# GestaltCogTeam/STEP

Measured on AMD Instinct MI355X. Metric: training windows/sec on PEMS04, horizon-12 MAE parity, 1/2/4/8 MI355X, higher is better.
Workload: dtype f16 (TSFormer Q/K/weights) + bf16 (P, V, GraphWaveNet / graph-learner GEMMs) operands, f32 accumulate

## Files before the change

include/step_hip.h:

```cpp
#ifndef STEP_HIP_H
#define STEP_HIP_H

#include <stdint.h>

#ifdef __cplusplus
extern "C" {
#endif

const char* step_last_error(void);
int step_abi_version(void);

typedef struct StepGemm {
    int M, N, K, batch;
    const void* A; long sam, sak, sab; int a_bf16;
    const void* B; long sbk, sbn, sbb; int b_bf16;
    float* C; long ldc, scn, scb;
    float alpha;
    int accumulate;
    const float* bias; int relu;
    int splitk;
    int a_kblk; long a_kstride;
    int b_kblk; long b_kstride;
    int b_nblk; long b_nstride;
    int c_nblk; long c_nstride;
// ... 8 lines not shown
int step_gemm(const StepGemm* g, void* stream);

#define STEP_ENC_F16 1
#define STEP_ENC_ALWAYS_RESHIFT 2
#define STEP_ENC_RANGE_FLAG 4
#define STEP_ENC_WORKGROUPS(n) (((n) & 0xffff) << 8)
int step_tsformer_encode(const float* series, int S, int L, const void* wpack, long wpack_bytes,
                         int depth, int flags, uint16_t* hidden_bf16, float* hidden_f32, float* last_f32,
                         float* sqnorm_part, float dropout_p, const uint64_t* drop_pool, long pool_words, uint64_t seed,
                         unsigned int* fallback_count, void* stream);
int step_dropout_pool_fill(uint64_t* pool, long words, float dropout_p, uint64_t seed, void* stream);
long step_tsformer_dropout_words(int L, int depth);

int step_pack_long_history(const float* x, int B, int L, int N, int C, int ch, float* out, void* stream);
int step_gather_windows(const float* data, int T, int N, int C, int ch, const long* t0, int B, int L, int H,
                        float* long_series, float* hist, float* fut, void* stream);

long step_knn_workspace_bytes(int B, int N, int F);
int step_knn_graph(const uint16_t* hidden, const float* sqnorm_part, int B, int N, int F, int k_total,
                   float* sim, float* adj, void* work, long work_bytes, void* stream);
int step_topk_mask(const float* sim, int B, int N, int k_total, float* adj, void* work, long work_bytes,
                   void* stream);

typedef struct StepDglParams {
    float *conv1_w, *conv1_b;
    float *conv2_w, *conv2_b;
    float *fc_w, *fc_b;
    float *bn1_w, *bn1_b, *bn1_rm, *bn1_rv;
    float *bn2_w, *bn2_b, *bn2_rm, *bn2_rv;
    float *bn3_w, *bn3_b, *bn3_rm, *bn3_rv;
    float *fc_out_w, *fc_out_b;
    float *fc_cat_w, *fc_cat_b;
    int gemm_bf16;
} StepDglParams;

long step_dgl_global_saved_floats(int N, int T);
long step_dgl_global_work_floats(int N, int T, int backward);
int step_dgl_global_forward(const float* series_nt, int N, int T, const StepDglParams* p, int training,
                            float momentum, float* saved, float* work, float* g, void* stream);
int step_dgl_global_backward(const float* series_nt, int N, int T, const StepDglParams* p, const float* saved,
                             const float* dg, float* work, const StepDglParams* grads, void* stream);
#define STEP_DGL_FRESH_FC_GRAD 16
int step_dgl_global_backward_phase(const float* series_nt, int N, int T, const StepDglParams* p, const float* saved,
                             const float* dg, float* work, const StepDglParams* grads, int phase, void* stream);

typedef struct StepDglShard { int own1; double count1, count2; } StepDglShard;
int step_dgl_global_forward_shard(const float* series_slice, int N, int Ts, const StepDglParams* p, int training, float momentum,
                                  float* saved, float* work, double* sums, float* g, const StepDglShard* shard, int phase,
                                  void* stream);
int step_dgl_global_backward_shard(const float* series_slice, int N, int Ts, const StepDglParams* p, const float* saved,
                                   const float* dg, float* work, const StepDglParams* grads, const StepDglShard* shard, int phase,
                                   void* stream);
long step_dgl_global_offset(int N, int T, int item);

long step_dgl_edges_saved_floats(int B, int N);
long step_dgl_edges_work_floats(int N);
long step_dgl_edges_theta_offset(int N);
int step_dgl_edges_forward(const float* g, int N, int B, const StepDglParams* p, const float* u, uint64_t seed,
                           float temperature, float* saved, float* theta_out, float* adj_out, void* stream);
int step_dgl_edges_backward(const float* g, int N, int B, const StepDglParams* p, const float* saved,
                            const float* dtheta, const float* dadj, float temperature, float* work,
                            const StepDglParams* grads, float* dg, void* aux_stream, void* stream);

typedef struct StepGwnetParams {
    float *nodevec1, *nodevec2;
    float *start_w, *start_b;
    float *filter_w[8], *filter_b[8];
    float *gate_w[8], *gate_b[8];
    float *skip_w[8], *skip_b[8];
    float *bn_w[8], *bn_b[8], *bn_rm[8], *bn_rv[8];
    float *gconv_w[8], *gconv_b[8];
    float *fc_his0_w, *fc_his0_b, *fc_his2_w, *fc_his2_b;
    float *end1_w, *end1_b, *end2_w, *end2_b;
    int gemm_bf16;
} StepGwnetParams;

long step_gwnet_saved_floats(int B, int N, int dropout);
long step_gwnet_work_floats(int B, int N, int backward);
long step_gwnet_saved_offset(int B, int N, int dropout, int item, int layer);
int step_gwnet_forward(const float* hist, int B, int N, int Cin, const float* hidden_last, const float* adj,
                       const StepGwnetParams* p, int training, float dropout_p, uint64_t seed, float momentum,
                       float* saved, float* work, float* pred, void* stream);
int step_gwnet_forward_phase(const float* hist, int B, int N, int Cin, const float* hidden_last, const float* adj,
                             const StepGwnetParams* p, int training, float dropout_p, uint64_t seed, float momentum,
                             float* saved, float* work, float* pred, int phase, void* stream);
int step_gwnet_backward(const float* hist, int B, int N, int Cin, const float* hidden_last, const StepGwnetParams* p,
                        const float* saved, float* work, const float* dpred, const StepGwnetParams* grads,
                        float* dadj, int dropout, void* aux_stream, void* leaf_stream, void* stream);

int step_pt_dropout(const float* x, float* y, long n, float p, uint64_t seed, uint32_t site, void* stream);
int step_pt_ffn_hidden_fwd(const float* x, const float* w1, const float* b1, long R, float p, uint64_t seed, uint32_t site,
                           uint16_t* hidden, void* stream);
int step_pt_ffn_hidden_bwd(const float* dy, const float* w2, const uint16_t* hidden, long R, float p, uint16_t* dhidden, void* stream);
int step_pt_colsum_bf16(const uint16_t* x, long rows, int cols, float* out, void* stream);
long step_pt_rows_linear_pack_bytes(int nkc, int nog);
int step_pt_rows_linear_pack(const float* w, long swo, long swi, int nkc, int nog, const float* bias, void* pack, void* stream);
int step_pt_rows_linear(const void* x, int x_bf16, long R, const void* pack, int nkc, int nog, void* y, int y_bf16, int accumulate, void* stream);
int step_pt_layer_pack(const float* wi, const float* bi, const float* wo, const float* bo, const float* w1, const float* b1, const float* w2,
                       const float* b2, void* ffn, void* qkv, void* o, void* da, void* dx, void* stream);
long step_pt_proj_wgrad_ws_floats(long R);
int step_pt_proj_wgrad(const float* x, const uint16_t* dqkv, const float* dov, const uint16_t* a, long R, float* ws, float* dwi, float* dbi, float* dwo,
                       void* stream);
int step_pt_ffn_fused_fwd_ln(const float* h1, long R, const void* pack, float p, const uint64_t* pool, long pool_words, uint64_t seed, uint32_t site_hidden,
                             uint32_t site_out, const float* gamma, const float* beta, float* pre, float* y, float* stats, void* stream);
int step_pt_rows_linear_ln(const uint16_t* x, long R, const void* pack, const float* res, float p, uint64_t seed, uint32_t site, const float* gamma,
                           const float* beta, float* pre, float* y, float* stats, void* stream);
// ... 129 lines not shown
```

step_amd/_lib.py:

```python
import ctypes
import os

import torch

_HERE = os.path.dirname(os.path.abspath(__file__))
LIB_PATH = os.environ.get("STEP_HIP_LIB") or os.path.join(_HERE, "libstep_hip.so")

_vp, _i, _l, _f, _u64 = ctypes.c_void_p, ctypes.c_int, ctypes.c_long, ctypes.c_float, ctypes.c_uint64


class StepGemm(ctypes.Structure):
    _fields_ = [("M", _i), ("N", _i), ("K", _i), ("batch", _i),
                ("A", _vp), ("sam", _l), ("sak", _l), ("sab", _l), ("a_bf16", _i),
                ("B", _vp), ("sbk", _l), ("sbn", _l), ("sbb", _l), ("b_bf16", _i),
                ("C", _vp), ("ldc", _l), ("scn", _l), ("scb", _l),
                ("alpha", _f), ("accumulate", _i), ("bias", _vp), ("relu", _i), ("splitk", _i),
                ("a_kblk", _i), ("a_kstride", _l), ("b_kblk", _i), ("b_kstride", _l),
                ("b_nblk", _i), ("b_nstride", _l), ("c_nblk", _i), ("c_nstride", _l),
                ("a_kscale", _vp), ("a_kshift", _vp), ("a_kperiod", _i),
                ("batch0", _i), ("sab1", _l), ("sbb1", _l), ("scb1", _l), ("compute_bf16", _i), ("a_rowsum", _vp), ("c_nscale", _vp), ("c_nshift", _vp), ("c_mvec", _vp),
                ("c_nperiod", _i), ("splitk_ws", _vp), ("splitk_ws_floats", _l)]


class StepDglParams(ctypes.Structure):
    NAMES = ["conv1_w", "conv1_b", "conv2_w", "conv2_b", "fc_w", "fc_b",
             "bn1_w", "bn1_b", "bn1_rm", "bn1_rv", "bn2_w", "bn2_b", "bn2_rm", "bn2_rv",
             "bn3_w", "bn3_b", "bn3_rm", "bn3_rv", "fc_out_w", "fc_out_b", "fc_cat_w", "fc_cat_b"]
    _fields_ = [(n, _vp) for n in NAMES] + [("gemm_bf16", _i)]


class StepGwnetParams(ctypes.Structure):
    _fields_ = [("nodevec1", _vp), ("nodevec2", _vp), ("start_w", _vp), ("start_b", _vp),
                ("filter_w", _vp * 8), ("filter_b", _vp * 8), ("gate_w", _vp * 8), ("gate_b", _vp * 8),
                ("skip_w", _vp * 8), ("skip_b", _vp * 8),
                ("bn_w", _vp * 8), ("bn_b", _vp * 8), ("bn_rm", _vp * 8), ("bn_rv", _vp * 8),
                ("gconv_w", _vp * 8), ("gconv_b", _vp * 8),
                ("fc_his0_w", _vp), ("fc_his0_b", _vp), ("fc_his2_w", _vp), ("fc_his2_b", _vp),
                ("end1_w", _vp), ("end1_b", _vp), ("end2_w", _vp), ("end2_b", _vp), ("gemm_bf16", _i)]


_PD = ctypes.POINTER(StepDglParams)


class StepDynState(ctypes.Structure):
    _fields_ = [("seed_xor", ctypes.c_uint64), ("adam_step", ctypes.c_int32), ("lr", _f), ("gsl_coef", _f), ("reserved", _f)]


class StepDglShard(ctypes.Structure):
    _fields_ = [("own1", ctypes.c_int), ("count1", ctypes.c_double), ("count2", ctypes.c_double)]


_PS = ctypes.POINTER(StepDglShard)
_PG = ctypes.POINTER(StepGwnetParams)

_SIGS = {
    "step_last_error": (ctypes.c_char_p, []),
    "step_abi_version": (_i, []),
    "step_gemm": (_i, [ctypes.POINTER(StepGemm), _vp]),
    "step_tsformer_encode": (_i, [_vp, _i, _i, _vp, _l, _i, _i, _vp, _vp, _vp, _vp, _f, _vp, _l, _u64, _vp, _vp]),
    "step_dropout_pool_fill": (_i, [_vp, _l, _f, _u64, _vp]),
    "step_tsformer_dropout_words": (_l, [_i, _i]),
    "step_gather_windows": (_i, [_vp, _i, _i, _i, _i, _vp, _i, _i, _i, _vp, _vp, _vp, _vp]),
    "step_pack_long_history": (_i, [_vp, _i, _i, _i, _i, _i, _vp, _vp]),
    "step_knn_workspace_bytes": (_l, [_i, _i, _i]),
    "step_knn_graph": (_i, [_vp, _vp, _i, _i, _i, _i, _vp, _vp, _vp, _l, _vp]),
    "step_topk_mask": (_i, [_vp, _i, _i, _i, _vp, _vp, _l, _vp]),
    "step_selftest_mfma": (_i, [_vp, _vp]),
    "step_streams_concurrent": (_i, [_vp, _vp, ctypes.POINTER(_i)]),
    "step_dgl_global_saved_floats": (_l, [_i, _i]),
    "step_dgl_global_work_floats": (_l, [_i, _i, _i]),
    "step_dgl_global_forward": (_i, [_vp, _i, _i, _PD, _i, _f, _vp, _vp, _vp, _vp]),
    "step_dgl_global_backward": (_i, [_vp, _i, _i, _PD, _vp, _vp, _vp, _PD, _vp]),
    "step_dgl_global_backward_phase": (_i, [_vp, _i, _i, _PD, _vp, _vp, _vp, _PD, _i, _vp]),
    "step_dgl_global_forward_shard": (_i, [_vp, _i, _i, _PD, _i, _f, _vp, _vp, _vp, _vp, _PS, _i, _vp]),
    "step_dgl_global_backward_shard": (_i, [_vp, _i, _i, _PD, _vp, _vp, _vp, _PD, _PS, _i, _vp]),
    "step_dgl_global_offset": (_l, [_i, _i, _i]),
    "step_dgl_edges_saved_floats": (_l, [_i, _i]),
    "step_dgl_edges_work_floats": (_l, [_i]),
    "step_dgl_edges_theta_offset": (_l, [_i]),
    "step_dgl_edges_forward": (_i, [_vp, _i, _i, _PD, _vp, _u64, _f, _vp, _vp, _vp, _vp]),
    "step_dgl_edges_backward": (_i, [_vp, _i, _i, _PD, _vp, _vp, _vp, _f, _vp, _PD, _vp, _vp, _vp]),
    "step_gwnet_saved_floats": (_l, [_i, _i, _i]),
    "step_gwnet_work_floats": (_l, [_i, _i, _i]),
    "step_gwnet_saved_offset": (_l, [_i, _i, _i, _i, _i]),
    "step_gwnet_forward": (_i, [_vp, _i, _i, _i, _vp, _vp, _PG, _i, _f, _u64, _f, _vp, _vp, _vp, _vp]),
    "step_gwnet_forward_phase": (_i, [_vp, _i, _i, _i, _vp, _vp, _PG, _i, _f, _u64, _f, _vp, _vp, _vp, _i, _vp]),
    "step_gwnet_backward": (_i, [_vp, _i, _i, _i, _vp, _PG, _vp, _vp, _vp, _PG, _vp, _i, _vp, _vp, _vp]),
    "step_pt_dropout": (_i, [_vp, _vp, _l, _f, _u64, ctypes.c_uint32, _vp]),
    "step_pt_ffn_hidden_fwd": (_i, [_vp, _vp, _vp, _l, _f, _u64, ctypes.c_uint32, _vp, _vp]),
    "step_pt_ffn_hidden_bwd": (_i, [_vp, _vp, _vp, _l, _f, _vp, _vp]),
    "step_pt_colsum_bf16": (_i, [_vp, _l, _i, _vp, _vp]),
    "step_pt_rows_linear_pack_bytes": (_l, [_i, _i]),
    "step_pt_rows_linear_pack": (_i, [_vp, _l, _l, _i, _i, _vp, _vp, _vp]),
    "step_pt_rows_linear": (_i, [_vp, _i, _l, _vp, _i, _i, _vp, _i, _i, _vp]),
    "step_pt_layer_pack": (_i, [_vp] * 14),
    "step_pt_proj_wgrad_ws_floats": (_l, [_l]),
    "step_pt_proj_wgrad": (_i, [_vp, _vp, _vp, _vp, _l, _vp, _vp, _vp, _vp, _vp]),
    "step_pt_ffn_fused_fwd_ln": (_i, [_vp, _l, _vp, _f, _vp, _l, _u64, ctypes.c_uint32, ctypes.c_uint32, _vp, _vp, _vp, _vp, _vp, _vp]),
    "step_pt_rows_linear_ln": (_i, [_vp, _l, _vp, _vp, _f, _u64, ctypes.c_uint32, _vp, _vp, _vp, _vp, _vp, _vp]),
    "step_pt_embed_unmasked_fwd": (_i, [_vp, _vp, _vp, _vp, _vp, _l, _i, _i, _f, _u64, ctypes.c_uint32, _vp, _vp]),
    "step_pt_embed_unmasked_bwd": (_i, [_vp, _vp, _vp, _l, _i, _i, _f, _u64, ctypes.c_uint32, _vp, _vp, _vp, _vp]),
    "step_pt_dec_input_bwd_sums": (_i, [_vp, _l, _i, _i, _f, _u64, ctypes.c_uint32, _vp, _vp, _vp, _vp, _vp]),
    "step_pt_ffn_pack_bytes": (_l, []),
    "step_pt_ffn_wgrad_workgroups": (_l, [_l]),
    "step_pt_ffn_wgrad_ws_floats": (_l, [_l]),
    "step_pt_ffn_pack": (_i, [_vp, _vp, _vp, _vp, _vp, _vp]),
    "step_pt_ffn_fused_fwd": (_i, [_vp, _l, _vp, _f, _vp, _l, _u64, ctypes.c_uint32, _vp, _vp]),
    "step_pt_ffn_fused_bwd_data": (_i, [_vp, _vp, _l, _vp, _f, _vp, _l, _u64, ctypes.c_uint32, _vp, _vp]),
    "step_pt_ffn_fused_bwd_weights": (_i, [_vp, _vp, _l, _vp, _vp, _f, _vp, _l, _u64, ctypes.c_uint32, _vp, _vp, _vp, _vp, _vp]),
    "step_pt_add_layernorm_fwd": (_i, [_vp, _vp, _l, _f, _u64, ctypes.c_uint32, _vp, _vp, _vp, _vp, _vp, _vp]),
    "step_pt_layernorm_bwd_dropout": (_i, [_vp, _vp, _l, _vp, _vp, _vp, _vp, _f, _u64, ctypes.c_uint32, _vp, _vp, _vp, _vp]),
    "step_pt_dropout_relu_mask": (_i, [_vp, _vp, _l, _f, _u64, ctypes.c_uint32, _vp]),
    "step_pt_add_dropout": (_i, [_vp, _vp, _vp, _l, _f, _u64, ctypes.c_uint32, _vp]),
    "step_pt_add_rows": (_i, [_vp, _l, _i, _vp, _vp, _vp]),
    "step_pt_sum_over_seq": (_i, [_vp, _l, _i, _i, _i, _vp, _vp, _vp]),
    "step_pt_token_gather": (_i, [_vp, _l, _i, _vp, _i, _f, _vp, _vp]),
    "step_pt_token_scatter": (_i, [_vp, _l, _i, _vp, _i, _f, _vp, _vp]),
    "step_pt_dec_input": (_i, [_vp, _vp, _vp, _vp, _l, _i, _i, _f, _u64, ctypes.c_uint32, _vp, _vp]),
    "step_pt_dec_input_bwd": (_i, [_vp, _l, _i, _i, _f, _u64, ctypes.c_uint32, _vp, _vp, _vp]),
    "step_pt_layernorm_fwd": (_i, [_vp, _l, _vp, _vp, _vp, _vp, _vp]),
    "step_pt_layernorm_bwd": (_i, [_vp, _vp, _l, _vp, _vp, _vp, _vp, _vp, _vp]),
    "step_pt_attention_fwd": (_i, [_vp, _l, _i, _f, _u64, ctypes.c_uint32, _vp, _vp, _vp]),
    "step_pt_attention_bwd": (_i, [_vp, _vp, _vp, _vp, _l, _i, _f, _u64, ctypes.c_uint32, _vp, _vp]),
    "step_pt_attention_fwd_bf16": (_i, [_vp, _l, _i, _f, _u64, ctypes.c_uint32, _vp, _vp, _vp, _vp, _l, _vp]),
    "step_pt_attention_bwd_bf16": (_i, [_vp, _vp, _vp, _vp, _l, _i, _f, _u64, ctypes.c_uint32, _vp, _vp, _vp]),
    "step_pt_linear_bf16out": (_i, [_vp, _vp, _l, _l, _vp, _l, _i, _i, _vp, _vp]),
    "step_pt_relu_mask": (_i, [_vp, _vp, _l, _vp]),
    "step_colsum": (_i, [_vp, _l, _i, _l, _vp, _vp]),
    "step_loss_fwd_bwd": (_i, [_vp, _vp, _l, _vp, _vp, _l, _f, _f, _vp, _vp, _vp, _vp, _vp]),
# ... 118 lines not shown
```

step_amd/build.py:

```python
import os
import subprocess
import sys

HERE = os.path.dirname(os.path.abspath(__file__))
CSRC = os.path.join(HERE, "csrc")
LIB = os.path.join(HERE, "libstep_hip.so")
SOURCES = ["errors.cpp", "comm.cpp", "gemm.hip", "gemm_bf16.hip", "tsformer_encoder.hip", "knn.hip", "selftest.hip",
           "dgl.hip", "dgl_conv_mfma.hip", "gwnet.hip", "optim.hip", "pretrain.hip", "pretrain_fused.hip", "pretrain_attn2.hip",
           "eval_cache.hip", "eval_metrics.hip", "train_tail.hip", "pretrain_tail.hip", "replica_digest.hip"]


def _newer(target, deps):
    if not os.path.exists(target):
        return True
    t = os.path.getmtime(target)
    return any(os.path.getmtime(d) > t for d in deps)


def build(force=False, verbose=True):
    hipcc = os.environ.get("HIPCC", "/opt/rocm/bin/hipcc")
    srcs = [os.path.join(CSRC, s) for s in SOURCES if os.path.exists(os.path.join(CSRC, s))]
    hdrs = [os.path.join(CSRC, f) for f in os.listdir(CSRC) if f.endswith(".h")]
    hdrs.append(os.path.join(HERE, "..", "include", "step_hip.h"))
    objs = []
    os.makedirs(os.path.join(HERE, "build"), exist_ok=True)
    procs = []
    for s in srcs:
        o = os.path.join(HERE, "build", os.path.basename(s) + ".o")
        objs.append(o)
        if force or _newer(o, [s] + hdrs):
            cmd = [hipcc, "--offload-arch=gfx950", "-O3", "-std=c++17", "-fPIC", "-x", "hip", "-c", s, "-o", o]
            if verbose:
                print(" ".join(cmd), flush=True)
            procs.append((s, subprocess.Popen(cmd, stdout=subprocess.PIPE, stderr=subprocess.STDOUT)))
    for s, p in procs:
        out, _ = p.communicate()
        if p.returncode != 0:
            sys.stderr.write(out.decode())
            raise RuntimeError("hipcc failed on " + s)
    if force or _newer(LIB, objs):
        cmd = [hipcc, "--offload-arch=gfx950", "-shared", "-fPIC", "-o", LIB] + objs + ["-ldl"]
        if verbose:
            print(" ".join(cmd), flush=True)
        subprocess.check_call(cmd)
    return LIB


if __name__ == "__main__":
    build(force="--force" in sys.argv)
```

step_amd/csrc/dgl.hip:

```cpp
#include "common.h"
#include "step_internal.h"

namespace {

constexpr int KW = 10;
constexpr int EMB = 100;

template <int CI, int CO, int TPT>
__global__ __launch_bounds__(256) void conv_relu_fwd_kernel(const float* __restrict__ in, const float* __restrict__ w,
                                                            const float* __restrict__ b, const float* __restrict__ in_sc,
                                                            const float* __restrict__ in_sh, float* __restrict__ out,
                                                            float* __restrict__ partial, int Tin, int stat_limit) {
    __shared__ __attribute__((aligned(16))) float ws[CI * KW * CO];
    __shared__ float red[4][2 * CO];
    const int tid = threadIdx.x, n = blockIdx.y;
    const int Tout = Tin - (KW - 1);
    for (int e = tid; e < CI * KW * CO; e += 256) {
        int co = e % CO, k = (e / CO) % KW, ci = e / (CO * KW);
        ws[e] = w[(co * CI + ci) * KW + k];
    }
    __syncthreads();
    const int t0 = (blockIdx.x * 256 + tid) * TPT;
    float acc[CO][TPT];
#pragma unroll
// ... 541 lines not shown
    } else {
        const float s = sndT[(long)f * N + j];
        float a = 0.f;
#pragma unroll 8
        for (int i = 0; i < N; ++i) {
            float hid = rcv[(long)i * EMB + f] + s;
            float d = dz[(long)i * N + j];
            a += hid > 0.f ? d : 0.f;
        }
        dsndT[(long)f * N + j] = a * wd;
    }
}

__global__ void colsum_kernel(const float* __restrict__ x, long rows, int cols, long ld, float* __restrict__ out) {
    __shared__ float red[4][64];
    const int c = blockIdx.x * 64 + (threadIdx.x & 63);
    const int w = threadIdx.x >> 6;
    float s = 0.f;
    if (c < cols)
        for (long r = (long)blockIdx.y * 4 + w; r < rows; r += (long)gridDim.y * 4) s += x[r * ld + c];
    red[w][threadIdx.x & 63] = s;
    __syncthreads();
    if (w == 0 && c < cols) atomicAdd(&out[c], red[0][threadIdx.x] + red[1][threadIdx.x] + red[2][threadIdx.x] + red[3][threadIdx.x]);
}

}

int step_colsum_launch(const float* x, long rows, int cols, long ld, float* out, hipStream_t st) {
    int chunks = (int)((rows + 255) / 256);
    if (chunks > 512) chunks = 512;
    if (chunks < 1) chunks = 1;
    colsum_kernel<<<dim3(cdiv(cols, 64), chunks), 256, 0, st>>>(x, rows, cols, ld, out);
    STEP_LAUNCH_CHECK("colsum");
    return STEP_OK;
}

constexpr int DGL_SMALL = 256 + 64 + 1344 + 100 * 32;

__global__ void bn2_fused_coef_kernel(const float* __restrict__ dots, const float* __restrict__ stat, const float* __restrict__ gamma,
                                      double count, float* __restrict__ dgamma, float* __restrict__ dbeta, float* __restrict__ coef) {
    constexpr int C = 16;
    const int c = threadIdx.x;
    if (c >= C) return;
    const float S1 = dots[2 * c + 1];
    const float S2 = stat[3 * C + c] * (dots[2 * c] - stat[2 * C + c] * S1);
    dgamma[c] += S2;
    dbeta[c] += S1;
    coef[c] = (float)(S1 / count);
    coef[C + c] = (float)(S2 / count);
    coef[2 * C + c] = gamma[c] * stat[3 * C + c];
}

__global__ __launch_bounds__(256) void fc_prep_kernel(const float* __restrict__ fc_w, const float* __restrict__ st2, uint4* __restrict__ wp,
                                                      float* __restrict__ shiftdot, int T2) {
    __shared__ float red[4];
    const int o = blockIdx.y, t = blockIdx.x * 256 + threadIdx.x, tid = threadIdx.x;
    float acc = 0.f;
    if (t < T2) {
        float v[16];
#pragma unroll
        for (int c = 0; c < 16; ++c) v[c] = fc_w[((long)o * 16 + c) * T2 + t];
#pragma unroll
        for (int c = 0; c < 16; ++c) { acc += v[c] * st2[16 + c]; v[c] *= st2[c]; }
        uint4* dst = wp + ((long)o * T2 + t) * 2;
        dst[0] = make_uint4(pack_bf16x2(v[0], v[1]), pack_bf16x2(v[2], v[3]), pack_bf16x2(v[4], v[5]), pack_bf16x2(v[6], v[7]));
        dst[1] = make_uint4(pack_bf16x2(v[8], v[9]), pack_bf16x2(v[10], v[11]), pack_bf16x2(v[12], v[13]), pack_bf16x2(v[14], v[15]));
    }
    acc = wave_sum(acc);
    if ((tid & 63) == 0) red[tid >> 6] = acc;
    __syncthreads();
    if (tid == 0) atomicAdd(&shiftdot[o], red[0] + red[1] + red[2] + red[3]);
}
__global__ void gpre_init_kernel(float* __restrict__ gpre, const float* __restrict__ shiftdot, long n) {
    const long i = (long)blockIdx.x * 256 + threadIdx.x;
    if (i < n) gpre[i] = shiftdot[i % EMB];
}
__global__ __launch_bounds__(256) void fc_unpermute_kernel(const float* __restrict__ graw, const float* __restrict__ fc_w,
                                                           const float* __restrict__ st2, const float* __restrict__ colsum,
                                                           float* __restrict__ dfc_w, float* __restrict__ dots_o, int T2, int overwrite) {
    __shared__ float red[16][32];
    const int o = blockIdx.y, t = blockIdx.x * 256 + threadIdx.x, tid = threadIdx.x, lane = tid & 63, wave = tid >> 6;
    const float cso = colsum[o];
    float d[32];
#pragma unroll
    for (int i = 0; i < 32; ++i) d[i] = 0.f;
    if (t < T2) {
        const float4* src = (const float4*)(graw + ((long)o * T2 + t) * 16);
        const float4 g0 = src[0], g1 = src[1], g2 = src[2], g3 = src[3];
        const float g[16] = {g0.x, g0.y, g0.z, g0.w, g1.x, g1.y, g1.z, g1.w, g2.x, g2.y, g2.z, g2.w, g3.x, g3.y, g3.z, g3.w};
        float w[16], old[16];
#pragma unroll
        for (int c = 0; c < 16; ++c) { const long idx = ((long)o * 16 + c) * T2 + t; w[c] = fc_w[idx]; old[c] = overwrite ? 0.f : dfc_w[idx]; }
#pragma unroll
        for (int c = 0; c < 16; ++c) {
            dfc_w[((long)o * 16 + c) * T2 + t] = old[c] + st2[c] * g[c] + st2[16 + c] * cso;
            d[2 * c] = w[c] * g[c]; d[2 * c + 1] = w[c] * cso;
        }
    }
#pragma unroll
    for (int i = 0; i < 32; ++i) {
        const float v = row_sum_fast(d[i]);
        if ((lane & 15) == 15) red[4 * wave + (lane >> 4)][i] = v;
    }
    __syncthreads();
    if (tid < 32) {
        float v = 0.f;
#pragma unroll
        for (int r = 0; r < 16; ++r) v += red[r][tid];
        atomicAdd(&dots_o[o * 32 + tid], v);
    }
}
__global__ void dots_reduce_kernel(const float* __restrict__ dots_o, float* __restrict__ dots) {
    const int i = threadIdx.x;
    if (i >= 32) return;
    double a = 0.0;
    for (int o = 0; o < EMB; ++o) a += dots_o[o * 32 + i];
    dots[i] = (float)a;
}

static bool dgl_channels_last(const StepDglParams* p) {
    const char* e = getenv("STEP_DGL_F32_STORAGE");
    return p->gemm_bf16 && !(e && e[0] == '1');
}

static bool dgl_legacy_bn_backward() {
    const char* e = getenv("STEP_DGL_LEGACY_BN");
    return e && e[0] == '1';
}

extern "C" long step_dgl_global_saved_floats(int N, int T) {
    long T1 = T - 9, T2 = T - 18;
    return (long)N * 8 * T1 + (long)N * 16 * T2 + (long)N * EMB + 4 * 8 + 4 * 16 + 4 * EMB + (long)EMB * 16 * T2 + 128;
}
static long fc_splitk_ws_floats(int N, int T2) {
    const int splits = step_gemm_auto_splitk(N, EMB, 16 * T2, 1);
    return splits > 1 ? (long)splits * N * EMB + 4 : 0;
}
static long wraw_floats(long T2) {
    const long w = (long)EMB * 16 * T2, pack = dgl_conv2_pack_floats();
    return w > pack ? w : pack;
}
extern "C" long step_dgl_global_work_floats(int N, int T, int backward) {
    long T1 = T - 9, T2 = T - 18;
    long nb1 = (long)N * cdiv(T1, 1024), nb2 = (long)N * cdiv(T2, 1024);
    long part = (nb1 > nb2 ? nb1 : nb2) * 32 + 64;
    if (!backward) return part + dgl_conv2_pack_floats() + 64 + fc_splitk_ws_floats(N, (int)T2);
    return part + (long)N * 16 * T2 + (long)N * 8 * T1 + wraw_floats(T2) + 2L * N * EMB + DGL_SMALL + dgl_conv2_wgrad_scratch_floats(N, (int)T1);
}

static float* saved_wp(float* saved, int N, int T) {
    long T1 = T - 9, T2 = T - 18;
    return saved + (long)N * 8 * T1 + (long)N * 16 * T2 + (long)N * EMB + 4 * 8 + 4 * 16 + 4 * EMB;
}
static void carve_saved(float* saved, int N, int T, float** a1, float** a2, float** gpre, float** st1, float** st2, float** st3) {
    long T1 = T - 9, T2 = T - 18;
    *a1 = saved; saved += (long)N * 8 * T1;
    *a2 = saved; saved += (long)N * 16 * T2;
    *gpre = saved; saved += (long)N * EMB;
    *st1 = saved; saved += 4 * 8;
    *st2 = saved; saved += 4 * 16;
    *st3 = saved;
}

static int dgl_bn_stats(const float* partial, int nblk, int C, double count, const float* gamma, const float* beta, float* rm, float* rv,
                        int training, float momentum, float* stat, double* sums, hipStream_t st) {
    if (nblk < 8192) {
        bn_finalize_kernel<<<C, 256, 0, st>>>(partial, nblk, C, count, gamma, beta, rm, rv, training, momentum, stat);
    } else {
        if (hipMemsetAsync(sums, 0, 2 * C * sizeof(double), st) != hipSuccess) { step_set_error("memset failed"); return STEP_ERR_HIP; }
        bn_sums_sliced_kernel<<<dim3(C, 32), 256, 0, st>>>(partial, nblk, C, sums);
        bn_finalize_sums_kernel<<<1, 64, 0, st>>>(sums, C, count, gamma, beta, rm, rv, training, momentum, stat);
    }
    STEP_LAUNCH_CHECK("bn_stats");
    return STEP_OK;
}

static int dgl_global_forward_impl(const float* series_nt, int N, int T, const StepDglParams* p, int training, float momentum,
                                   float* saved, float* work, double* sums, float* g, const StepDglShard* shard, int phase,
                                   hipStream_t st) {
    const int T1 = T - 9, T2 = T - 18;
    float *a1, *a2, *gpre, *st1, *st2, *st3;
    carve_saved(saved, N, T, &a1, &a2, &gpre, &st1, &st2, &st3);
    float* partial = work;
    const bool all = phase == 0;
    const double count1 = shard ? shard->count1 : (double)N * T1, count2 = shard ? shard->count2 : (double)N * T2;
    const bool cl = dgl_channels_last(p);
    const long part_floats = ((long)N * cdiv(T1, 1024) > (long)N * cdiv(T2, 1024) ? (long)N * cdiv(T1, 1024) : (long)N * cdiv(T2, 1024)) * 32 + 64;
    double* own_sums = (double*)(work + part_floats + dgl_conv2_pack_floats());
    float* wp = saved_wp(saved, N, T);
    float* shiftdot = wp + (long)EMB * 16 * T2;
    if (all || phase == 1) {
        int nblk;
        if (cl) {
            STEP_TRY(dgl_conv1_fwd_cl(series_nt, p->conv1_w, p->conv1_b, a1, partial, N, T, shard ? shard->own1 : T1, &nblk, st));
        } else {
            dim3 grid(cdiv(T1, 256 * 4), N);
            conv_relu_fwd_kernel<1, 8, 4><<<grid, 256, 0, st>>>(series_nt, p->conv1_w, p->conv1_b, nullptr, nullptr, a1, partial, T,
                                                                shard ? shard->own1 : T1);
            STEP_LAUNCH_CHECK("conv1");
            nblk = grid.x * grid.y;
        }
        if (shard) bn_sums_kernel<<<8, 256, 0, st>>>(partial, nblk, 8, sums);
        else STEP_TRY(dgl_bn_stats(partial, nblk, 8, count1, p->bn1_w, p->bn1_b, p->bn1_rm, p->bn1_rv, training, momentum, st1, own_sums, st));
        STEP_LAUNCH_CHECK("bn1");
    }
    if (all || phase == 2) {
        if (shard) bn_finalize_sums_kernel<<<1, 64, 0, st>>>(sums, 8, count1, p->bn1_w, p->bn1_b, p->bn1_rm, p->bn1_rv, training, momentum, st1);
        int nblk;
        if (cl) {
            STEP_TRY(dgl_conv2_fwd_cl(a1, p->conv2_w, p->conv2_b, st1, st1 + 8, a2, partial, N, T1, &nblk,
                                      work + part_floats, st));
        } else if (p->gemm_bf16) {
            STEP_TRY(dgl_conv2_fwd_mfma(a1, p->conv2_w, p->conv2_b, st1, st1 + 8, a2, partial, N, T1, &nblk, st));
        } else {
            dim3 grid(cdiv(T2, 256 * 4), N);
            conv_relu_fwd_kernel<8, 16, 4><<<grid, 256, 0, st>>>(a1, p->conv2_w, p->conv2_b, st1, st1 + 8, a2, partial, T1, T2);
            STEP_LAUNCH_CHECK("conv2");
            nblk = grid.x * grid.y;
        }
        if (shard) bn_sums_kernel<<<16, 256, 0, st>>>(partial, nblk, 16, sums + 16);
        else STEP_TRY(dgl_bn_stats(partial, nblk, 16, count2, p->bn2_w, p->bn2_b, p->bn2_rm, p->bn2_rv, training, momentum, st2, own_sums, st));
        STEP_LAUNCH_CHECK("bn2");
    }
    if (all || phase == 3) {
        if (shard) bn_finalize_sums_kernel<<<1, 64, 0, st>>>(sums + 16, 16, count2, p->bn2_w, p->bn2_b, p->bn2_rm, p->bn2_rv, training, momentum, st2);
        const long K = 16L * T2;
        StepGemm gm = gemm_desc(N, EMB, (int)K, a2, K, 1, p->fc_w, 1, K, gpre, EMB);
        if (cl) {
            if (hipMemsetAsync(shiftdot, 0, 128 * sizeof(float), st) != hipSuccess) { step_set_error("memset failed"); return STEP_ERR_HIP; }
            fc_prep_kernel<<<dim3(cdiv(T2, 256), EMB), 256, 0, st>>>(p->fc_w, st2, (uint4*)wp, shiftdot, T2);
            gpre_init_kernel<<<cdiv((long)N * EMB, 256), 256, 0, st>>>(gpre, shiftdot, (long)N * EMB);
            STEP_LAUNCH_CHECK("fc_prep");
            gm.a_bf16 = 1;
            gm.B = wp; gm.b_bf16 = 1;
        } else {
            if (hipMemsetAsync(gpre, 0, (size_t)N * EMB * sizeof(float), st) != hipSuccess) { step_set_error("memset failed"); return STEP_ERR_HIP; }
            gm.a_kscale = st2; gm.a_kshift = st2 + 16; gm.a_kperiod = T2;
        }
        gm.accumulate = 2;
        gm.splitk = -1;
        gm.compute_bf16 = p->gemm_bf16;
        if (fc_splitk_ws_floats(N, T2) > 0) {
            float* ws = work + part_floats + dgl_conv2_pack_floats() + 64;
            gm.splitk_ws = (float*)(((uintptr_t)ws + 15) & ~(uintptr_t)15);
            gm.splitk_ws_floats = fc_splitk_ws_floats(N, T2) - 4;
        }
        STEP_TRY(step_gemm_launch(gm, st));
    }
    if (all || phase == 4) {
        fc_post_bn3_kernel<<<EMB, 256, 0, st>>>(gpre, p->fc_b, N, p->bn3_w, p->bn3_b, p->bn3_rm, p->bn3_rv, training, momentum, st3, g);
        STEP_LAUNCH_CHECK("fc_post_bn3");
    }
    return STEP_OK;
}

extern "C" int step_dgl_global_forward(const float* series_nt, int N, int T, const StepDglParams* p, int training,
                                       float momentum, float* saved, float* work, float* g, void* stream) {
    STEP_REQUIRE(series_nt && p && saved && work && g && N > 0 && T > 18, "dgl_global_forward: bad arguments");
    return dgl_global_forward_impl(series_nt, N, T, p, training, momentum, saved, work, nullptr, g, nullptr, 0, (hipStream_t)stream);
}

extern "C" int step_dgl_global_forward_shard(const float* series_slice, int N, int Ts, const StepDglParams* p, int training,
                                             float momentum, float* saved, float* work, double* sums, float* g,
                                             const StepDglShard* shard, int phase, void* stream) {
    STEP_REQUIRE(series_slice && p && saved && work && sums && g && shard && N > 0 && Ts > 18 && phase >= 1 && phase <= 4,
                 "dgl_global_forward_shard: bad arguments");
    STEP_REQUIRE(shard->own1 > 0 && shard->own1 <= Ts - 9 && shard->count1 > 0 && shard->count2 > 0, "dgl_global_forward_shard: bad shard");
    return dgl_global_forward_impl(series_slice, N, Ts, p, training, momentum, saved, work, sums, g, shard, phase, (hipStream_t)stream);
}

extern "C" long step_dgl_global_offset(int N, int T, int item) {
    const long T1 = T - 9, T2 = T - 18;
    if (item == 0) return 0;
    if (item == 1) return (long)N * 8 * T1;
    if (item == 2) return (long)N * 8 * T1 + (long)N * 16 * T2;
    const long nb1 = (long)N * cdiv(T1, 1024), nb2 = (long)N * cdiv(T2, 1024);
    const long coef = (nb1 > nb2 ? nb1 : nb2) * 32 + 64 + (long)N * 16 * T2 + (long)N * 8 * T1 + wraw_floats(T2) + 2L * N * EMB;
    if (item == 10) return coef + 256;
    if (item == 11) return coef + 320;
    return -1;
}

static int dgl_global_backward_impl(const float* series_nt, int N, int T, const StepDglParams* p, const float* saved, const float* dg,
                                    float* work, const StepDglParams* grads, const StepDglShard* shard, int phase, void* stream);

extern "C" int step_dgl_global_backward(const float* series_nt, int N, int T, const StepDglParams* p, const float* saved,
                                        const float* dg, float* work, const StepDglParams* grads, void* stream) {
    return step_dgl_global_backward_phase(series_nt, N, T, p, saved, dg, work, grads, 0, stream);
}

extern "C" int step_dgl_global_backward_phase(const float* series_nt, int N, int T, const StepDglParams* p, const float* saved,
                                              const float* dg, float* work, const StepDglParams* grads, int phase, void* stream) {
    STEP_REQUIRE(series_nt && p && saved && dg && work && grads && N > 0 && T > 18 && (phase & ~STEP_DGL_FRESH_FC_GRAD) >= 0 &&
                 (phase & ~STEP_DGL_FRESH_FC_GRAD) <= 2, "dgl_global_backward: bad arguments");
    return dgl_global_backward_impl(series_nt, N, T, p, saved, dg, work, grads, nullptr, phase, stream);
}

extern "C" int step_dgl_global_backward_shard(const float* series_slice, int N, int Ts, const StepDglParams* p, const float* saved,
                                              const float* dg, float* work, const StepDglParams* grads, const StepDglShard* shard,
                                              int phase, void* stream) {
// ... 223 lines not shown
```

step_amd/csrc/step_internal.h:

```cpp
#pragma once
#include <hip/hip_runtime.h>
#include <vector>
#include "../../include/step_hip.h"

enum { GEMM_FUSED_INTERLEAVED = 1, GEMM_FUSED_FFN_FWD = 2, GEMM_FUSED_MASKNZ = 4, GEMM_FUSED_BF16OUT = 8 };
struct GemmFused {
    const float* dotw; float* dots;
    const float* bnx; const float* bncoef; const float* bnstat;
    int channels, period;
    int flags;
    const float* ffn_bias; const void* maskx; float p; unsigned seed_lo, seed_hi, site;
};

struct GemmKSeg { long a_off, b_off, a_bs, b_bs; int a_rs, b_rs; };
constexpr int GEMM_KSEG_MAX = 128;
int step_gemm_segmented_launch(StepGemm g, const GemmKSeg* ktab, int ktab_per, hipStream_t st);

int step_gemm_launch(StepGemm g, hipStream_t st);
int step_gemm_auto_splitk(int M, int N, int K, int batch);
int step_gemm_launch_fused(StepGemm g, const GemmFused& fused, hipStream_t st);
int step_gemm_bf16_launch(StepGemm g, hipStream_t st, const GemmFused* fused = nullptr);
int step_gemm_f32_fast_launch(StepGemm g, hipStream_t st, const GemmFused* fused = nullptr);

static inline StepGemm gemm_desc(int M, int N, int K, const float* A, long sam, long sak, const float* B, long sbk,
                                 long sbn, float* C, long ldc) {
    StepGemm g;
    memset(&g, 0, sizeof(g));
    g.M = M; g.N = N; g.K = K; g.batch = 1;
    g.A = A; g.sam = sam; g.sak = sak;
    g.B = B; g.sbk = sbk; g.sbn = sbn;
    g.C = C; g.ldc = ldc; g.scn = 1;
    g.alpha = 1.f; g.splitk = 1;
    return g;
}

int step_gemm_rowsum_separate(StepGemm* g, hipStream_t st);
int dgl_conv2_fwd_mfma(const float* a1, const float* w, const float* b, const float* sc, const float* sh, float* a2, float* partial,
                       int N, int T1, int* nblk, hipStream_t st);
int dgl_conv2_dgrad_mfma(const float* dz, const float* w, float* din, int N, int T1, const float* bnx, const float* coef, const float* stat,
                         int own, hipStream_t st);
int dgl_conv2_wgrad_xhat_mfma(const float* dz, const float* a1, const float* stat1, float* scratch, float* graw, int N, int T1, hipStream_t st);
int dgl_conv2_wgrad_finish(const float* graw, const float* w, const float* stat1, const float* gamma1, const float* beta1, double count,
                           float* dw, float* db, float* dgamma1, float* dbeta1, float* coef1, int raw, hipStream_t st);
int dgl_conv1_fwd_cl(const float* x, const float* w, const float* b, void* a1h, float* partial, int N, int T, int stat_limit, int* nblk,
                     hipStream_t st);
long dgl_conv2_pack_floats();
int dgl_conv2_fwd_cl(const void* a1h, const float* w, const float* b, const float* sc, const float* sh, void* a2h, float* partial, int N,
                     int T1, int* nblk, float* pack, hipStream_t st);
int dgl_conv2_dgrad_cl(const void* dz2h, const float* w, const float* sc, void* dz1h, int N, int T1, const void* a1h, const float* coef,
                       const float* stat, int own, float* pack, hipStream_t st);
int dgl_conv2_wgrad_cl(const void* dz2h, const void* a1h, float* scratch, float* graw, int N, int T1, hipStream_t st);
int dgl_conv1_wgrad_cl(const void* dz1h, const float* x, float* scratch, float* dw, float* db, int N, int T, hipStream_t st);
long dgl_conv2_wgrad_scratch_floats(int N, int T1);
int dgl_conv2_wgrad_mfma(const float* dz, const float* a1, const float* sc, const float* sh, float* scratch, float* dw, float* db, int N,
                         int T1, hipStream_t st);
int dgl_conv1_wgrad_mfma(const float* dz, const float* x, float* scratch, float* dw, float* db, int N, int T, hipStream_t st);
int step_colsum_launch(const float* x, long rows, int cols, long ld, float* out, hipStream_t st);

struct AuxLane {
    hipStream_t main, aux;
    bool on;
    int next = 0, base = 0;
    AuxLane(hipStream_t m, hipStream_t a, int base_ = 0) : main(m), aux(a), on(a != nullptr && a != m), base(base_) {}
    static hipEvent_t event(int k) {
        thread_local std::vector<hipEvent_t> pool[16];
        int dev = 0;
        (void)hipGetDevice(&dev);
        std::vector<hipEvent_t>& v = pool[dev & 15];
        while ((int)v.size() <= k) {
            hipEvent_t e;
            if (hipEventCreateWithFlags(&e, hipEventDisableTiming) != hipSuccess) return nullptr;
            v.push_back(e);
        }
        return v[k];
    }
    hipStream_t fork() {
        if (!on) return main;
        hipEvent_t e = event(base + (next++ & 63));
        if (!e || hipEventRecord(e, main) != hipSuccess || hipStreamWaitEvent(aux, e, 0) != hipSuccess) { on = false; return main; }
        return aux;
    }
    hipEvent_t mark() {
        if (!on) return nullptr;
        hipEvent_t e = event(base + (next++ & 63));
        if (!e || hipEventRecord(e, main) != hipSuccess) { on = false; return nullptr; }
        return e;
    }
    hipStream_t after(hipEvent_t e) {
        if (!on || !e) return main;
        if (hipStreamWaitEvent(aux, e, 0) != hipSuccess) { on = false; return main; }
        return aux;
    }
    hipEvent_t done() {
        if (!on) return nullptr;
        hipEvent_t e = event(base + (next++ & 63));
        if (!e || hipEventRecord(e, aux) != hipSuccess) return nullptr;
        return e;
    }
    int wait_done(hipEvent_t e) {
        if (!on) return STEP_OK;
        if (!e) return join();
        if (hipStreamWaitEvent(main, e, 0) != hipSuccess) { step_set_error("backward: stream join failed"); return STEP_ERR_HIP; }
        return STEP_OK;
    }
    int join() {
        if (!on) return STEP_OK;
// ... 9 lines not shown
```

Measured before the change: 2400.

## Add streamed split-K MFMA kernel for graph-learner FC forward GEMM

Replaces the generic split-K GEMM for the graph-learner FC layer (N nodes × 100 outputs, very long K = 16·T2) with a dedicated kernel. The kernel streams bf16 rows of both operands into LDS via global_load_lds with a 3-stage pipeline, splits K across many workgroups, and then runs a deterministic reduce kernel. The shift-dot term is written as per-block partials instead of atomics, which removes the memset, the gpre_init kernel and the atomic accumulation, and folds the bias shift into the reduce. In exchange it adds a larger workspace and inline-asm DMA code that only applies when N <= 320 and the operand pointers are aligned.

Result: no change. 2419, median of 6 (+0.8%).

```diff
diff --git a/include/step_hip.h b/include/step_hip.h
--- a/include/step_hip.h
+++ b/include/step_hip.h
@@ -84,6 +84,9 @@
                                    const float* dg, float* work, const StepDglParams* grads, const StepDglShard* shard, int phase,
                                    void* stream);
 long step_dgl_global_offset(int N, int T, int item);
+long step_dgl_fc_forward_work_floats(int N, int T2);
+int step_dgl_fc_forward(const void* a2_bf16, const void* wp_bf16, const float* shiftdot, int N, int T2, float* work, float* gpre,
+                        void* stream);
 
 long step_dgl_edges_saved_floats(int B, int N);
 long step_dgl_edges_work_floats(int N);
diff --git a/step_amd/_lib.py b/step_amd/_lib.py
--- a/step_amd/_lib.py
+++ b/step_amd/_lib.py
@@ -75,6 +75,8 @@
     "step_dgl_global_forward_shard": (_i, [_vp, _i, _i, _PD, _i, _f, _vp, _vp, _vp, _vp, _PS, _i, _vp]),
     "step_dgl_global_backward_shard": (_i, [_vp, _i, _i, _PD, _vp, _vp, _vp, _PD, _PS, _i, _vp]),
     "step_dgl_global_offset": (_l, [_i, _i, _i]),
+    "step_dgl_fc_forward_work_floats": (_l, [_i, _i]),
+    "step_dgl_fc_forward": (_i, [_vp, _vp, _vp, _i, _i, _vp, _vp, _vp]),
     "step_dgl_edges_saved_floats": (_l, [_i, _i]),
     "step_dgl_edges_work_floats": (_l, [_i]),
     "step_dgl_edges_theta_offset": (_l, [_i]),
diff --git a/step_amd/build.py b/step_amd/build.py
--- a/step_amd/build.py
+++ b/step_amd/build.py
@@ -6,7 +6,7 @@
 CSRC = os.path.join(HERE, "csrc")
 LIB = os.path.join(HERE, "libstep_hip.so")
 SOURCES = ["errors.cpp", "comm.cpp", "gemm.hip", "gemm_bf16.hip", "tsformer_encoder.hip", "knn.hip", "selftest.hip",
-           "dgl.hip", "dgl_conv_mfma.hip", "gwnet.hip", "optim.hip", "pretrain.hip", "pretrain_fused.hip", "pretrain_attn2.hip",
+           "dgl.hip", "dgl_conv_mfma.hip", "dgl_fc_stream.hip", "gwnet.hip", "optim.hip", "pretrain.hip", "pretrain_fused.hip", "pretrain_attn2.hip",
            "eval_cache.hip", "eval_metrics.hip", "train_tail.hip", "pretrain_tail.hip", "replica_digest.hip"]
 
 
diff --git a/step_amd/csrc/dgl.hip b/step_amd/csrc/dgl.hip
--- a/step_amd/csrc/dgl.hip
+++ b/step_amd/csrc/dgl.hip
@@ -617,7 +617,7 @@
 }
 
 __global__ __launch_bounds__(256) void fc_prep_kernel(const float* __restrict__ fc_w, const float* __restrict__ st2, uint4* __restrict__ wp,
-                                                      float* __restrict__ shiftdot, int T2) {
+                                                      float* __restrict__ shiftdot, float* __restrict__ shift_part, int T2) {
     __shared__ float red[4];
     const int o = blockIdx.y, t = blockIdx.x * 256 + threadIdx.x, tid = threadIdx.x;
     float acc = 0.f;
@@ -634,7 +634,11 @@
     acc = wave_sum(acc);
     if ((tid & 63) == 0) red[tid >> 6] = acc;
     __syncthreads();
-    if (tid == 0) atomicAdd(&shiftdot[o], red[0] + red[1] + red[2] + red[3]);
+    if (tid == 0) {
+        const float v = red[0] + red[1] + red[2] + red[3];
+        if (shift_part) shift_part[(long)o * gridDim.x + blockIdx.x] = v;
+        else atomicAdd(&shiftdot[o], v);
+    }
 }
 __global__ void gpre_init_kernel(float* __restrict__ gpre, const float* __restrict__ shiftdot, long n) {
     const long i = (long)blockIdx.x * 256 + threadIdx.x;
@@ -709,7 +713,11 @@
     long T1 = T - 9, T2 = T - 18;
     long nb1 = (long)N * cdiv(T1, 1024), nb2 = (long)N * cdiv(T2, 1024);
     long part = (nb1 > nb2 ? nb1 : nb2) * 32 + 64;
-    if (!backward) return part + dgl_conv2_pack_floats() + 64 + fc_splitk_ws_floats(N, (int)T2);
+    if (!backward) {
+        const long staged = fc_splitk_ws_floats(N, (int)T2);
+        const long stream = dgl_fc_stream_serves(N) ? dgl_fc_stream_ws_floats(N, (int)T2) + 4 + (long)EMB * cdiv(T2, 256) : 0;
+        return part + dgl_conv2_pack_floats() + 64 + (staged > stream ? staged : stream);
+    }
     return part + (long)N * 16 * T2 + (long)N * 8 * T1 + wraw_floats(T2) + 2L * N * EMB + DGL_SMALL + dgl_conv2_wgrad_scratch_floats(N, (int)T1);
 }
 
@@ -791,10 +799,13 @@
         if (shard) bn_finalize_sums_kernel<<<1, 64, 0, st>>>(sums + 16, 16, count2, p->bn2_w, p->bn2_b, p->bn2_rm, p->bn2_rv, training, momentum, st2);
         const long K = 16L * T2;
         StepGemm gm = gemm_desc(N, EMB, (int)K, a2, K, 1, p->fc_w, 1, K, gpre, EMB);
+        float* fc_ws = (float*)(((uintptr_t)(work + part_floats + dgl_conv2_pack_floats() + 64) + 15) & ~(uintptr_t)15);
+        const bool streamed = cl && dgl_fc_stream_serves(N) && ((((uintptr_t)a2) | ((uintptr_t)wp)) & 15) == 0;
         if (cl) {
-            if (hipMemsetAsync(shiftdot, 0, 128 * sizeof(float), st) != hipSuccess) { step_set_error("memset failed"); return STEP_ERR_HIP; }
-            fc_prep_kernel<<<dim3(cdiv(T2, 256), EMB), 256, 0, st>>>(p->fc_w, st2, (uint4*)wp, shiftdot, T2);
-            gpre_init_kernel<<<cdiv((long)N * EMB, 256), 256, 0, st>>>(gpre, shiftdot, (long)N * EMB);
+            float* shift_part = streamed ? fc_ws + dgl_fc_stream_ws_floats(N, T2) : nullptr;
+            if (!streamed && hipMemsetAsync(shiftdot, 0, 128 * sizeof(float), st) != hipSuccess) { step_set_error("memset failed"); return STEP_ERR_HIP; }
+            fc_prep_kernel<<<dim3(cdiv(T2, 256), EMB), 256, 0, st>>>(p->fc_w, st2, (uint4*)wp, shiftdot, shift_part, T2);
+            if (!streamed) gpre_init_kernel<<<cdiv((long)N * EMB, 256), 256, 0, st>>>(gpre, shiftdot, (long)N * EMB);
             STEP_LAUNCH_CHECK("fc_prep");
             gm.a_bf16 = 1;
             gm.B = wp; gm.b_bf16 = 1;
@@ -802,15 +813,18 @@
             if (hipMemsetAsync(gpre, 0, (size_t)N * EMB * sizeof(float), st) != hipSuccess) { step_set_error("memset failed"); return STEP_ERR_HIP; }
             gm.a_kscale = st2; gm.a_kshift = st2 + 16; gm.a_kperiod = T2;
         }
-        gm.accumulate = 2;
-        gm.splitk = -1;
-        gm.compute_bf16 = p->gemm_bf16;
-        if (fc_splitk_ws_floats(N, T2) > 0) {
-            float* ws = work + part_floats + dgl_conv2_pack_floats() + 64;
-            gm.splitk_ws = (float*)(((uintptr_t)ws + 15) & ~(uintptr_t)15);
-            gm.splitk_ws_floats = fc_splitk_ws_floats(N, T2) - 4;
-        }
-        STEP_TRY(step_gemm_launch(gm, st));
+        if (streamed) {
+            STEP_TRY(dgl_fc_stream_forward(a2, wp, nullptr, fc_ws + dgl_fc_stream_ws_floats(N, T2), cdiv(T2, 256), N, T2, fc_ws, gpre, st));
+        } else {
+            gm.accumulate = 2;
+            gm.splitk = -1;
+            gm.compute_bf16 = p->gemm_bf16;
+            if (fc_splitk_ws_floats(N, T2) > 0) {
+                gm.splitk_ws = fc_ws;
+                gm.splitk_ws_floats = fc_splitk_ws_floats(N, T2) - 4;
+            }
+            STEP_TRY(step_gemm_launch(gm, st));
+        }
     }
     if (all || phase == 4) {
         fc_post_bn3_kernel<<<EMB, 256, 0, st>>>(gpre, p->fc_b, N, p->bn3_w, p->bn3_b, p->bn3_rm, p->bn3_rv, training, momentum, st3, g);
diff --git a/step_amd/csrc/dgl_fc_stream.hip b/step_amd/csrc/dgl_fc_stream.hip
--- /dev/null
+++ b/step_amd/csrc/dgl_fc_stream.hip
@@ -0,0 +1,206 @@
+#include "common.h"
+#include "step_internal.h"
+
+namespace {
+
+constexpr int FS_EMB = 100;
+constexpr int FS_KS = 64, FS_ROWB = FS_KS * 2;
+constexpr int FS_STAGES = 3;
+constexpr int FS_MT_MAX = 10;
+constexpr int FS_SLICE_TARGET = 96;
+__host__ __device__ constexpr int fs_rows8(int MT) { return (FS_EMB + 32 * MT + 7) & ~7; }
+
+__device__ __forceinline__ void fs_dma_1k(const void* gsrc_lane, uint32_t lds_dst) {
+    uint32_t keep;
+    lds_dst = __builtin_amdgcn_readfirstlane(lds_dst);
+    asm volatile("s_mov_b32 %0, m0\n\ts_mov_b32 m0, %2\n\ts_nop 0\n\tglobal_load_lds_dwordx4 %1, off\n\ts_mov_b32 m0, %0"
+                 : "=&s"(keep)
+                 : "v"(gsrc_lane), "s"(lds_dst)
+                 : "memory");
+}
+
+template <int MT>
+__global__ __launch_bounds__(256) void fc_fwd_stream_kernel(const uint16_t* __restrict__ a2, const uint16_t* __restrict__ wp, int N, long K,
+                                                            int steps_per_slice, float* __restrict__ ws) {
+    extern __shared__ __attribute__((aligned(16))) char fs_lds[];
+    constexpr int R8 = fs_rows8(MT), G = R8 / 8, BUF = R8 * FS_ROWB, NJ = (G + 3) / 4, NJ_MIN = G / 4;
+    const int tid = threadIdx.x, lane = tid & 63, wave = __builtin_amdgcn_readfirstlane(tid >> 6);
+    const int row0 = blockIdx.x * 32 * MT, s = blockIdx.y;
+    const int nstep_all = (int)((K + FS_KS - 1) / FS_KS);
+    const int step0 = s * steps_per_slice;
+    const int nstep = min(nstep_all - step0, steps_per_slice);
+    const long pieces = K / 8;
+    f32x16 acc[MT];
+#pragma unroll
+    for (int t = 0; t < MT; ++t)
+#pragma unroll
+        for (int e = 0; e < 16; ++e) acc[t][e] = 0.f;
+    const uint32_t lds0 = (uint32_t)(uintptr_t)(__attribute__((address_space(3))) char*)fs_lds;
+    const int csw = (lane & 7) ^ ((lane >> 3) & 7);
+    const uint16_t* rowp[NJ];
+#pragma unroll
+    for (int j = 0; j < NJ; ++j) {
+        int lr = (wave + 4 * j) * 8 + (lane >> 3);
+        lr = lr < R8 ? lr : R8 - 1;
+        if (lr < FS_EMB) {
+            rowp[j] = wp + (long)lr * K;
+        } else {
+            int row = row0 + lr - FS_EMB;
+            row = row < N ? row : N - 1;
+            rowp[j] = a2 + (long)row * K;
+        }
+    }
+    auto issue = [&](int step, int buf) {
+        long pc = (long)(step0 + step) * (FS_KS / 8) + csw;
+        pc = pc < pieces ? pc : pieces - 1;
+#pragma unroll
+        for (int j = 0; j < NJ; ++j) {
+            const int g = wave + 4 * j;
+            if (j < NJ_MIN || g < G) fs_dma_1k(rowp[j] + pc * 8, lds0 + (uint32_t)(buf * BUF + g * 1024));
+        }
+    };
+    if (nstep > 0) {
+        const int r = lane & 31, h = lane >> 5;
+        issue(0, 0);
+        if (nstep > 1) issue(1, 1);
+        for (int i = 0; i < nstep; ++i) {
+            if (i + 1 < nstep) asm volatile("s_waitcnt vmcnt(%0)" ::"n"(NJ_MIN) : "memory");
+            else asm volatile("s_waitcnt vmcnt(0)" ::: "memory");
+            __syncthreads();
+            if (i + 2 < nstep) issue(i + 2, (i + 2) % FS_STAGES);
+            const char* buf = fs_lds + (i % FS_STAGES) * BUF;
+            const long kleft = K - (long)(step0 + i) * FS_KS;
+            const int nks = kleft >= FS_KS ? FS_KS / 16 : (int)(kleft / 16);
+            const char* pb = buf + (32 * wave + r) * FS_ROWB;
+            const char* pa = buf + (FS_EMB + r) * FS_ROWB;
+#pragma unroll
+            for (int ks = 0; ks < FS_KS / 16; ++ks) {
+                if (ks < nks) {
+                    const bf16x8 b = *(const bf16x8*)(pb + (((ks * 2 + h) ^ (r & 7)) << 4));
+                    const int sla = ((ks * 2 + h) ^ ((r + 4) & 7)) << 4;
+#pragma unroll
+                    for (int t = 0; t < MT; ++t) {
+                        const bf16x8 a = *(const bf16x8*)(pa + t * 32 * FS_ROWB + sla);
+                        acc[t] = __builtin_amdgcn_mfma_f32_32x32x16_bf16(a, b, acc[t], 0, 0, 0);
+                    }
+                }
+            }
+        }
+    }
+    if (32 * wave + (lane & 31) < FS_EMB) {
+        const long tiles = (long)gridDim.x * MT;
+#pragma unroll
+        for (int t = 0; t < MT; ++t) {
+            if (row0 + 32 * t < N) {
+                float* o = ws + (((long)s * tiles + blockIdx.x * MT + t) * 4 + wave) * 1024 + lane;
+#pragma unroll
+                for (int e = 0; e < 16; ++e) o[e * 64] = acc[t][e];
+            }
+        }
+    }
+}
+
+__global__ __launch_bounds__(256) void fc_fwd_reduce_kernel(const float* __restrict__ ws, const float* __restrict__ shiftdot,
+                                                            const float* __restrict__ shift_part, int nparts, int S, long tiles, int N,
+                                                            float* __restrict__ gpre) {
+    __shared__ float red[4][64];
+    __shared__ float sdp[8][32];
+    const int tid = threadIdx.x, lane = tid & 63, q = tid >> 6;
+    const long blk = blockIdx.x;
+    const int e = (int)(blk & 15), wv = (int)((blk >> 4) & 3);
+    const long tile = blk >> 6;
+    const long n = tile * 32 + 8 * (e >> 2) + (e & 3) + 4 * (lane >> 5);
+    const int o = wv * 32 + (lane & 31);
+    const bool ok = n < N && o < FS_EMB;
+    {
+        const int oc = wv * 32 + (tid & 31);
+        float sd = 0.f;
+        if (oc < FS_EMB) {
+            if (shiftdot) { if (tid < 32) sd = shiftdot[oc]; }
+            else for (int i = tid >> 5; i < nparts; i += 8) sd += shift_part[(long)oc * nparts + i];
+        }
+        sdp[tid >> 5][tid & 31] = sd;
+    }
+    float v[8];
+#pragma unroll
+    for (int c = 0; c < 8; ++c) v[c] = 0.f;
+    if (ok) {
+        const float* src = ws + blk * 64 + lane;
+        const long sstr = tiles * 4096;
+        for (int sp = q; sp < S; sp += 32) {
+#pragma unroll
+            for (int c = 0; c < 8; ++c) {
+                const int s2 = sp + 4 * c;
+                const float x = src[(long)(s2 < S ? s2 : S - 1) * sstr];
+                v[c] += s2 < S ? x : 0.f;
+            }
+        }
+    }
+    red[q][lane] = ((v[0] + v[1]) + (v[2] + v[3])) + ((v[4] + v[5]) + (v[6] + v[7]));
+    __syncthreads();
+    if (q == 0 && ok) {
+        const int c = lane & 31;
+        const float sd = ((sdp[0][c] + sdp[1][c]) + (sdp[2][c] + sdp[3][c])) + ((sdp[4][c] + sdp[5][c]) + (sdp[6][c] + sdp[7][c]));
+        gpre[n * FS_EMB + o] = sd + ((red[0][lane] + red[1][lane]) + (red[2][lane] + red[3][lane]));
+    }
+}
+
+struct FsPlan { int MT, RT, S, per; long tiles; };
+FsPlan fs_plan(int N, int T2) {
+    static const int forced = []() { const char* e = getenv("STEP_FC_STREAM_SLICES"); return e ? atoi(e) : 0; }();
+    FsPlan p;
+    const int tiles = (N + 31) / 32;
+    p.MT = tiles < FS_MT_MAX ? tiles : FS_MT_MAX;
+    p.RT = (tiles + p.MT - 1) / p.MT;
+    p.tiles = (long)p.RT * p.MT;
+    const int steps = (int)((16L * T2 + FS_KS - 1) / FS_KS);
+    int S = forced > 0 ? forced : (FS_SLICE_TARGET + p.RT - 1) / p.RT;
+    if (S > steps / 2) S = steps / 2;
+    if (S < 1) S = 1;
+    p.per = (steps + S - 1) / S;
+    p.S = (steps + p.per - 1) / p.per;
+    return p;
+}
+
+}
+
+bool dgl_fc_stream_serves(int N) {
+    static const bool off = []() { const char* e = getenv("STEP_FC_STREAM"); return e && e[0] == '0'; }();
+    return !off && N <= 32 * FS_MT_MAX;
+}
+
+long dgl_fc_stream_ws_floats(int N, int T2) {
+    const FsPlan p = fs_plan(N, T2);
+    return (long)p.S * p.tiles * 4096;
+}
+
+int dgl_fc_stream_forward(const void* a2, const void* wp, const float* shiftdot, const float* shift_part, int nparts, int N, int T2,
+                          float* ws, float* gpre, hipStream_t st) {
+    STEP_REQUIRE((((uintptr_t)a2 | (uintptr_t)wp) & 15) == 0, "dgl_fc_forward: the bf16 operands must be 16-byte aligned");
+    const FsPlan p = fs_plan(N, T2);
+    const long K = 16L * T2;
+    const dim3 grid(p.RT, p.S);
+    const int lds = FS_STAGES * fs_rows8(p.MT) * FS_ROWB;
+#define FS_LAUNCH(mt)                                                                                                       \
+    case mt:                                                                                                                \
+        STEP_TRY(step_raise_lds_once((const void*)fc_fwd_stream_kernel<mt>, 160 * 1024, "dgl_fc_forward"));                 \
+        fc_fwd_stream_kernel<mt><<<grid, 256, lds, st>>>((const uint16_t*)a2, (const uint16_t*)wp, N, K, p.per, ws);        \
+        break;
+    switch (p.MT) {
+        FS_LAUNCH(1) FS_LAUNCH(2) FS_LAUNCH(3) FS_LAUNCH(4) FS_LAUNCH(5) FS_LAUNCH(6) FS_LAUNCH(7) FS_LAUNCH(8) FS_LAUNCH(9) FS_LAUNCH(10)
+        default: STEP_REQUIRE(false, "dgl_fc_forward: %d row tiles per workgroup", p.MT);
+    }
+#undef FS_LAUNCH
+    STEP_LAUNCH_CHECK("fc_fwd_stream");
+    fc_fwd_reduce_kernel<<<(unsigned)(p.tiles * 64), 256, 0, st>>>(ws, shiftdot, shift_part, nparts, p.S, p.tiles, N, gpre);
+    STEP_LAUNCH_CHECK("fc_fwd_reduce");
+    return STEP_OK;
+}
+
+extern "C" long step_dgl_fc_forward_work_floats(int N, int T2) { return N > 0 && T2 > 0 ? dgl_fc_stream_ws_floats(N, T2) : 0; }
+
+extern "C" int step_dgl_fc_forward(const void* a2_bf16, const void* wp_bf16, const float* shiftdot, int N, int T2, float* work, float* gpre,
+                                   void* stream) {
+    STEP_REQUIRE(a2_bf16 && wp_bf16 && shiftdot && work && gpre && N > 0 && T2 > 0, "dgl_fc_forward: bad arguments");
+    return dgl_fc_stream_forward(a2_bf16, wp_bf16, shiftdot, nullptr, 0, N, T2, work, gpre, (hipStream_t)stream);
+}
diff --git a/step_amd/csrc/step_internal.h b/step_amd/csrc/step_internal.h
--- a/step_amd/csrc/step_internal.h
+++ b/step_amd/csrc/step_internal.h
@@ -52,6 +52,10 @@
 int dgl_conv2_wgrad_cl(const void* dz2h, const void* a1h, float* scratch, float* graw, int N, int T1, hipStream_t st);
 int dgl_conv1_wgrad_cl(const void* dz1h, const float* x, float* scratch, float* dw, float* db, int N, int T, hipStream_t st);
 long dgl_conv2_wgrad_scratch_floats(int N, int T1);
+bool dgl_fc_stream_serves(int N);
+long dgl_fc_stream_ws_floats(int N, int T2);
+int dgl_fc_stream_forward(const void* a2, const void* wp, const float* shiftdot, const float* shift_part, int nparts, int N, int T2,
+                          float* ws, float* gpre, hipStream_t st);
 int dgl_conv2_wgrad_mfma(const float* dz, const float* a1, const float* sc, const float* sh, float* scratch, float* dw, float* db, int N,
                          int T1, hipStream_t st);
 int dgl_conv1_wgrad_mfma(const float* dz, const float* x, float* scratch, float* dw, float* db, int N, int T, hipStream_t st);
```
